# danshapero/sigma

Hardware: AMD Instinct MI355X
Metric: SpMV GB/s (achieved HBM) + CG iters/sec on 5-pt Laplacian, N=1e7 (higher is better)
Workload: dtype f64; 1 GPU; 5-point 2D Poisson CSR, 3162x3162 rows per GPU (rank 0: n=9998244, nnz=49978572), fp64 SpMV y=A*x; rows_per_gpu=9998244, nnz_per_gpu=49978572, parallelism=row-partition x1, matrix_resident_bytes_per_gpu=479920788, reference_layout_bytes_per_gpu=639735844, full=False

## Files before the change

### sigma_amd/csrc/sgm_internal.hpp

```cpp
#pragma once
#include <hip/hip_runtime.h>

#include <cstdarg>
#include <cstdint>
#include <cstdio>
#include <cstring>
#include <string>
#include <atomic>
#include <type_traits>
#include <utility>
#include <vector>

#include "../../include/sigma_hip.h"

namespace sgm {

extern std::string g_err;
int fail(int code, const char *fmt, ...);

#define SGM_HIP(call)                                                              \
    do {                                                                           \
        hipError_t e__ = (call);                                                   \
        if (e__ != hipSuccess)                                                     \
            return sgm::fail(SGM_ERR_HIP, "%s:%d: %s -> %s", __FILE__, __LINE__,   \
                             #call, hipGetErrorString(e__));                       \
    } while (0)
#define SGM_TRY(call)                        \
    do {                                     \
        int rc__ = (call);                   \
        if (rc__ != SGM_OK) return rc__;     \
    } while (0)

constexpr int kEllcbMaxCols = 16384;
struct MatOptions {
    int csr_offset_dict = 1;
    int ell_offset_dict = 1;
    int csr_row_owner = 1;
    int csr_row_lines = 1;
    int csr_sliced = 1;
    int csr_sell = 1;
    int csr_xwindow = 1;
    int csr_lean = 1;
    int ell_colblock = 1;
    int ell_colblock_cols = 16384;
    int ell_colblock_rows = 0;
    int coloring_pass = 0;
    int slice_sched = 0;
};
struct SolverOptions {
    int cg_small = 1;
    int bicgstab_small = 1;
    int krylov_graph = 1;
    int dot_order = 0;
    int gmres_cgs2 = 1;
    int coop_spin_limit = 0;
    int cg_coop_variant = 0;
    int reorder_solve = 2;
    int dist_halo_fused = 1;
};
struct PcOptions {
    int ildu_strips = 1;
    int ildu_rows = 1;
    int pipeline_spin_limit = 0;
    int ildu_reorder = 0;
};
struct Options { MatOptions mat; SolverOptions solver; PcOptions pc; };
int *mat_option_field(MatOptions &o, const char *name);
int *solver_option_field(SolverOptions &o, const char *name);
int *pc_option_field(PcOptions &o, const char *name);
int normalise_option(const char *name, int value, int *out);
extern Options g_opt;

struct Runtime {
    bool ready = false;
// ... 59 lines not shown
    const double *ptr;
    int count;
};

struct HaloNbr {
    int peer = -1;
    int32_t send_count = 0;
    int32_t *send_idx = nullptr;
    double *send_buf = nullptr;
    int32_t recv_offset = 0;
    int32_t recv_count = 0;
};

struct SliceSched { int32_t *tab = nullptr; int32_t lo = 0, hi = 0, grid = 0, iters = 0, band = 0; };

struct Part {
    MatOptions opt = g_opt.mat;
    int32_t n = 0;
    int32_t ncol_own = 0;
    int32_t n_halo = 0;
    int32_t int_lo = 0, int_hi = 0;
    int64_t nnz = 0;
    int64_t row_begin = 0;
    int32_t *rowptr = nullptr;
    int32_t *col = nullptr;
    double *val = nullptr;
    uint8_t *code = nullptr;
    int32_t *dict = nullptr;
    int32_t ndict = 0;
    int32_t dict_reach = 0;
    int32_t max_row = 0;
    double *sval = nullptr;
    uint32_t *scode = nullptr;
    int32_t *scol = nullptr;
    uint8_t *sbcode = nullptr;
    bool lean = false;
    double *sl_val = nullptr;
    int32_t *sl_col = nullptr;
    uint16_t *sl_perm = nullptr;
    int64_t *sl_off = nullptr;
    int64_t sl_total = 0;
    int32_t *sl_win0 = nullptr;
    int32_t sl_gs = 1;
    int32_t sl_span = 0;
    int32_t sw = 0;
    int32_t sched_period = 0;
    mutable SliceSched sched[3];
    mutable int nsched = 0;
    const int32_t *run_sched = nullptr;
    int32_t run_iters = 0;
    int32_t max_d = 0;
    int32_t *ecol = nullptr;
    double *eval = nullptr;
    int32_t *edeg = nullptr;
    uint8_t *ezero = nullptr;
    uint8_t *ecode = nullptr;
    int32_t emdp = 0;
    int32_t *cb_perm = nullptr;
    double *cb_sval = nullptr;
    uint16_t *cb_lcol = nullptr;
    int32_t *cb_bstart = nullptr;
    uint16_t *cb_lpos = nullptr;
    void *cb_fdesc = nullptr;
    double *cb_P = nullptr;
    int32_t cb_cols = 0, cb_nb = 0, cb_R = 0, cb_ntiles = 0, cb_chunks = 0;
    int32_t cb_maxd = 0;
// ... 276 lines not shown
```

### sigma_amd/csrc/sgm_layouts.hip

```cpp
#include "sgm_spmv_select.hpp"

namespace sgm {

__global__ void k_dec1(int32_t *a, int64_t n)
{
    int64_t i = (int64_t)blockIdx.x * blockDim.x + threadIdx.x;
    const int64_t stride = (int64_t)gridDim.x * blockDim.x;
    for (; i < n; i += stride) a[i] -= 1;
}

__global__ void k_check_ptr1(const int32_t *__restrict__ ptr1, int64_t n, int64_t nnz, unsigned long long *bad)
{
    int64_t i = (int64_t)blockIdx.x * blockDim.x + threadIdx.x;
    const int64_t stride = (int64_t)gridDim.x * blockDim.x;
    for (; i <= n; i += stride) {
        const int32_t a = ptr1[i];
        bool ok = true;
        if (i == 0) ok = a == 1;
        if (i < n) ok = ok && ptr1[i + 1] >= a;
        else ok = ok && (int64_t)a - 1 == nnz;
        if (!ok) atomicMin(bad, (unsigned long long)i);
    }
}

// ... 245 lines not shown
{
    if (!p.lean || p.val) return SGM_OK;
    SGM_TRY(dalloc(&p.val, (size_t)p.nnz + 2));
    SGM_HIP(hipMemsetAsync(p.val + p.nnz, 0, 2 * sizeof(double), g_rt.stream));
    return SGM_OK;
}
void csr_release_arrays(const Part &cp)
{
    Part &p = const_cast<Part &>(cp);
    if (!p.lean || !lean_applies(p)) return;
    (void)hipStreamSynchronize(g_rt.stream);
    dfree(p.val); dfree(p.col); dfree(p.code);
    p.val = nullptr; p.col = nullptr; p.code = nullptr;
}

int pack_sliced(Part &p)
{
    if (p.sl_val && p.n > 0) {
        const int64_t nch = (((int64_t)p.n + kSlRows - 1) / kSlRows) * (kSlRows / kSellChunk);
        hipLaunchKernelGGL(k_sell_fill, dim3((unsigned)std::min<int64_t>((nch + 3) / 4, 65536)), dim3(256), 0, g_rt.stream, p.n,
                           (const int32_t *)p.rowptr, (const int32_t *)nullptr, (const double *)p.val, (const int64_t *)p.sl_off,
                           (const uint16_t *)p.sl_perm, (int32_t *)nullptr, p.sl_val);
        SGM_HIP(hipGetLastError());
    }
    if ((!p.scode && !p.scol && !p.sbcode) || p.n == 0) return SGM_OK;
    const int64_t nsl = ((int64_t)p.n + kSlRows - 1) / kSlRows;
    if (p.ecol)
        hipLaunchKernelGGL(k_sl_pack_ell, dim3((unsigned)std::min<int64_t>(nsl, 65536)), dim3(256), 0, g_rt.stream, p.n, p.sw,
                           p.max_d, (const double *)p.eval, p.sval);
    else
        hipLaunchKernelGGL(k_sl_pack, dim3((unsigned)std::min<int64_t>(nsl, 65536)), dim3(256), 0, g_rt.stream, p.n, p.sw,
                           (const int32_t *)p.rowptr, (const double *)p.val, p.sval);
    SGM_HIP(hipGetLastError());
    return SGM_OK;
}

__global__ void k_fill32(int64_t n, int32_t *a, int32_t v)
{
    int64_t i = (int64_t)blockIdx.x * blockDim.x + threadIdx.x;
    const int64_t stride = (int64_t)gridDim.x * blockDim.x;
    for (; i < n; i += stride) a[i] = v;
}

constexpr int kDictSlots = 1024;
constexpr int32_t kDictEmpty = INT32_MIN;
__global__ __launch_bounds__(256) void k_dict_collect(int32_t n, const int32_t *__restrict__ rowptr, const int32_t *__restrict__ col,
                                                      int32_t *table, int *count, int *max_row)
{
    constexpr int kLocal = 512;
    __shared__ int32_t ltab[kLocal];
    __shared__ int lcount;
    for (int t = threadIdx.x; t < kLocal; t += 256) ltab[t] = kDictEmpty;
    if (threadIdx.x == 0) lcount = 0;
    __syncthreads();
    int mr = 0;
    int32_t mine[8];
#pragma unroll
    for (int t = 0; t < 8; ++t) mine[t] = kDictEmpty;
    int next = 0;
    for (int32_t i = blockIdx.x * blockDim.x + threadIdx.x; i < n; i += gridDim.x * blockDim.x) {
        const int32_t s0 = rowptr[i], e = rowptr[i + 1];
        mr = max(mr, e - s0);
        for (int32_t k = s0; k < e; ++k) {
            const int32_t off = col[k] - i;
            bool known = false;
#pragma unroll
// ... 182 lines not shown
        SGM_TRY(build_ell_colblock(p));
        if (p.cb_P) return SGM_OK;
        const int W = p.max_row <= 3 ? 3 : p.max_row <= 5 ? 5 : p.max_row <= 7 ? 7 : p.max_row <= 8 ? 8 : p.max_row <= 12 ? 12
                    : p.max_row <= 16 ? 16 : p.max_row <= 20 ? 20 : p.max_row <= 24 ? 24 : p.max_row <= 28 ? 28 : 32;
        if (!p.opt.csr_sliced || p.max_row < 1 || p.max_row > 32 || (double)W * n > 1.25 * (double)nnz) return build_sell(p);
        const size_t rows_padded = ((size_t)n + kSlRows - 1) / kSlRows * kSlRows;
        SGM_TRY(dalloc(&p.scol, rows_padded * W));
        SGM_TRY(dalloc(&p.sval, rows_padded * W));
        p.sw = W;
        hipLaunchKernelGGL(k_sl_pack_cols, dim3((unsigned)std::min<size_t>(rows_padded / kSlRows, 65536)), dim3(256), 0, g_rt.stream,
                           n, W, (const int32_t *)p.rowptr, (const int32_t *)p.col, p.scol);
        SGM_HIP(hipGetLastError());
        return pack_sliced(p);
    };
    if (!p.opt.csr_offset_dict || hcnt[0] > 255) return sliced32();
    std::vector<int32_t> dict;
    for (int32_t v : htab) if (v != kDictEmpty) dict.push_back(v);
    std::sort(dict.begin(), dict.end());
    p.ndict = (int32_t)dict.size();
    p.dict_reach = 0;
    for (int32_t v : dict) p.dict_reach = std::max(p.dict_reach, v < 0 ? -v : v);
    dict.resize(256, 0);
    SGM_TRY(dalloc(&p.code, (size_t)nnz + 32));
    SGM_TRY(dalloc(&p.dict, (size_t)256));
    SGM_HIP(hipMemcpyAsync(p.dict, dict.data(), 256 * 4, hipMemcpyHostToDevice, st));
    SGM_HIP(hipMemsetAsync(p.code + nnz, 0, 32, st));
    const int W = p.max_row <= 3 ? 3 : p.max_row <= 5 ? 5 : p.max_row <= 7 ? 7 : 8;
    const bool sliced = p.opt.csr_sliced && p.ndict <= 15 && p.max_row >= 1 && p.max_row <= 8 && (double)W * n <= 1.25 * (double)nnz;
    size_t rows_padded = 0;
    if (sliced) {
        rows_padded = ((size_t)n + kSlRows - 1) / kSlRows * kSlRows;
        SGM_TRY(dalloc(&p.scode, rows_padded));
        SGM_TRY(dalloc(&p.sval, rows_padded * W));
        hipLaunchKernelGGL(k_fill32, dim3(vec_grid(rows_padded)), dim3(256), 0, st, (int64_t)rows_padded,
                           reinterpret_cast<int32_t *>(p.scode), (int32_t)-1);
        p.sw = W;
    }
    hipLaunchKernelGGL(k_dict_encode, dim3(grid), dim3(256), 0, st, n, (const int32_t *)p.rowptr, (const int32_t *)p.col,
                       (const int32_t *)p.dict, p.ndict, p.code, sliced ? p.scode : nullptr);
    SGM_HIP(hipGetLastError());
    if (sliced) SGM_TRY(pack_sliced(p));
    int Wb = 0;
#define PICK(WW) if (!Wb && p.max_row <= WW) Wb = WW;
    SGM_SLB_WIDTHS(PICK)
#undef PICK
    const int Wc = (Wb + 7) / 8 * 8;
    if (!sliced && p.opt.csr_sliced && Wb && p.ndict <= 255 && p.max_row > 8 && (double)Wb * n <= 1.35 * (double)nnz) {
        rows_padded = ((size_t)n + kSlRows - 1) / kSlRows * kSlRows;
        SGM_TRY(dalloc(&p.sbcode, rows_padded * Wc));
        SGM_TRY(dalloc(&p.sval, rows_padded * Wb));
        p.sw = Wb;
        hipLaunchKernelGGL(k_slb_pack_codes, dim3((unsigned)std::min<size_t>(rows_padded / kSlRows, 65536)), dim3(256), 0, st, n, Wb,
                           (const int32_t *)p.rowptr, (const uint8_t *)p.code, p.sbcode);
        SGM_HIP(hipGetLastError());
        SGM_TRY(pack_sliced(p));
    }
    SGM_HIP(hipStreamSynchronize(st));
    if (p.scode || p.sbcode) SGM_TRY(detect_sched_period_csr(p, dict));
    if (!p.scode && !p.sbcode) {
        SGM_TRY(build_sell(p));
        if (p.sl_val) {
            dfree(p.code); dfree(p.dict);
            p.code = nullptr; p.dict = nullptr;
            p.ndict = 0; p.dict_reach = 0;
        }
    }
// ... 200 lines not shown
        return fail(SGM_ERR_UNSUPPORTED, "clone_csr_plain: single-GPU CSR matrices only");
    const Part &p = A->parts[0];
    SGM_TRY(csr_need_arrays(p));
    struct Release { const Part &p; ~Release() { csr_release_arrays(p); } } rel{p};
    sgm_mat C = new sgm_mat_s;
    C->fmt = SGM_FMT_CSR; C->nrow = A->nrow; C->ncol = A->ncol; C->nnz = A->nnz;
    C->parts.resize(1);
    Part &q = C->parts[0];
    q.opt.csr_offset_dict = 0; q.opt.csr_sliced = 0; q.opt.csr_sell = 0; q.opt.csr_lean = 0; q.opt.slice_sched = 0;
    q.n = p.n; q.ncol_own = p.ncol_own; q.n_halo = 0; q.nnz = p.nnz; q.max_row = p.max_row;
    hipStream_t st = g_rt.stream;
    int rc = dalloc(&q.rowptr, (size_t)p.n + 1);
    if (rc == SGM_OK) rc = dalloc(&q.col, (size_t)p.nnz + 4);
    if (rc == SGM_OK) rc = dalloc(&q.val, (size_t)p.nnz + 2);
    if (rc != SGM_OK) { sgm_mat_destroy(C); return rc; }
    (void)hipMemcpyAsync(q.rowptr, p.rowptr, ((size_t)p.n + 1) * 4, hipMemcpyDeviceToDevice, st);
    (void)hipMemsetAsync(q.col + p.nnz, 0, 16, st);
    (void)hipMemsetAsync(q.val + p.nnz, 0, 16, st);
    if (p.nnz) {
        (void)hipMemcpyAsync(q.col, p.col, (size_t)p.nnz * 4, hipMemcpyDeviceToDevice, st);
        (void)hipMemcpyAsync(q.val, p.val, (size_t)p.nnz * 8, hipMemcpyDeviceToDevice, st);
    }
    if (hipStreamSynchronize(st) != hipSuccess || hipGetLastError() != hipSuccess) { sgm_mat_destroy(C); return fail(SGM_ERR_HIP, "clone_csr_plain: copy failed"); }
    *out = C;
    return SGM_OK;
}

int rebuild_csr_formats(Part &p)
{
    SGM_TRY(csr_need_arrays(p));
    p.lean = false;
    dfree(p.code); dfree(p.dict); dfree(p.sval); dfree(p.scode); dfree(p.scol); dfree(p.sbcode);
    p.code = nullptr; p.dict = nullptr; p.sval = nullptr; p.scode = nullptr; p.scol = nullptr; p.sbcode = nullptr;
    free_sell(p);
    free_ell_colblock(p);
    p.ndict = 0; p.dict_reach = 0; p.sw = 0; p.max_row = 0; p.sched_period = 0;
    free_slice_sched(p);
    return build_offset_dict(p, nullptr, nullptr);
}
int rebuild_ell_formats(Part &p)
{
    dfree(p.ecode); dfree(p.dict); dfree(p.sval); dfree(p.scode);
    p.ecode = nullptr; p.dict = nullptr; p.dict_reach = 0; p.emdp = 0; p.sval = nullptr; p.scode = nullptr; p.sw = 0; p.sched_period = 0;
    free_slice_sched(p);
    SGM_TRY(build_ell_offset_dict(p));
    SGM_TRY(build_ell_colblock(p));
    return refresh_ell_colblock_values(p);
}
int sgm_invalidate_transpose(sgm_mat A)
{
    if (A->T) { sgm_mat_destroy(A->T); A->T = nullptr; }
    dfree(A->tperm);
    A->tperm = nullptr;
    A->t_stale = true;
    return SGM_OK;
}

void free_part(Part &p)
{
    dfree(p.rowptr); dfree(p.col); dfree(p.val); dfree(p.code); dfree(p.dict); dfree(p.sval); dfree(p.scode); dfree(p.scol); dfree(p.sbcode); dfree(p.ecol); dfree(p.eval); dfree(p.edeg); dfree(p.ezero); dfree(p.ecode); dfree(p.xext);
    for (auto &nb : p.nbrs) { dfree(nb.send_idx); dfree(nb.send_buf); }
    free_slice_sched(p);
    free_ell_colblock(p);
    free_sell(p);
    p = Part();
}

}
```

### sigma_amd/csrc/sgm_mat.hip

```cpp
#include "sgm_spmv_select.hpp"
#include "sgm_krylov.hpp"
#include "sgm_plan_host.hpp"

namespace sgm {

int stage_in(Staged &s, const double *v, int64_t n, int where, bool copy)
{
    if (where == SGM_DEVICE && (reinterpret_cast<uintptr_t>(v) & 15) == 0) {
        s.dev = const_cast<double *>(v);
        return SGM_OK;
    }
    SGM_TRY(dalloc(&s.dev, (size_t)n));
    s.owned = true;
    if (copy)
        SGM_HIP(hipMemcpyAsync(s.dev, v, (size_t)n * 8,
                               where == SGM_HOST ? hipMemcpyHostToDevice : hipMemcpyDeviceToDevice,
                               g_rt.stream));
    return SGM_OK;
}
int stage_out(const Staged &s, double *v, int64_t n, int where)
{
    if (!s.owned) return SGM_OK;
    SGM_HIP(hipMemcpyAsync(v, s.dev, (size_t)n * 8,
                           where == SGM_HOST ? hipMemcpyDeviceToHost : hipMemcpyDeviceToDevice,
// ... 453 lines not shown
    unsigned long long *bad = nullptr, hbad = ~0ull;
    SGM_TRY(dalloc(&deg, (size_t)std::max(n, 1)));
    int rc = dalloc(&bad, 1);
    if (rc == SGM_OK && hipMemsetAsync(bad, 0xff, sizeof hbad, st) != hipSuccess) rc = fail(SGM_ERR_HIP, "sgm_ell_set_degrees: memset");
    if (rc == SGM_OK && n &&
        hipMemcpyAsync(deg, degrees, (size_t)n * 4, where == SGM_HOST ? hipMemcpyHostToDevice : hipMemcpyDeviceToDevice, st) != hipSuccess)
        rc = fail(SGM_ERR_HIP, "sgm_ell_set_degrees: copy of degrees");
    if (rc == SGM_OK && n)
        hipLaunchKernelGGL(k_ell_check_degrees, dim3((n + kBlock - 1) / kBlock), dim3(kBlock), 0, st, n, p.max_d, (const int32_t *)deg,
                           (const uint8_t *)p.ezero, bad);
    if (rc == SGM_OK && (hipMemcpyAsync(&hbad, bad, sizeof hbad, hipMemcpyDeviceToHost, st) != hipSuccess ||
                         hipStreamSynchronize(st) != hipSuccess || hipGetLastError() != hipSuccess))
        rc = fail(SGM_ERR_HIP, "sgm_ell_set_degrees: check kernel failed");
    dfree(bad);
    if (rc == SGM_OK && hbad != ~0ull) {
        int32_t d = 0;
        (void)hipMemcpy(&d, deg + hbad, 4, hipMemcpyDeviceToHost);
        rc = fail(SGM_ERR_DIMS, "sgm_ell_set_degrees: degrees(%lld) = %d: outside 0..%d, or one of the first %d slots of that row holds no column",
                  (long long)hbad + 1, d, p.max_d, d);
    }
    if (rc != SGM_OK) { dfree(deg); return rc; }
    dfree(p.edeg);
    p.edeg = deg;
    A->version += 1;
    A->pattern_version += 1;
    return SGM_OK;
}

int sgm_mat_set_option(sgm_mat A, const char *name, int value)
{
    SGM_TRY(require_init());
    if (!A || !name) return fail(SGM_ERR_BAD_ARG, "sgm_mat_set_option: null argument");
    int v = 0;
    SGM_TRY(normalise_option(name, value, &v));
    MatOptions probe;
    if (!mat_option_field(probe, name)) return fail(SGM_ERR_BAD_ARG, "sgm_mat_set_option: '%s' is not a matrix option", name);
    if (A->fmt == SGM_FMT_COMPOSITE) {
        for (sgm_mat_s *B : A->blocks)
            if (B) SGM_TRY(sgm_mat_set_option(B, name, value));
        return SGM_OK;
    }
    const bool cb_shape = !strcmp(name, "ell_colblock_cols") || !strcmp(name, "ell_colblock_rows");
    for (Part &p : A->parts) {
        int *f = mat_option_field(p.opt, name);
        const int old = *f;
        *f = v;
        if (old == v) continue;
        if ((p.ecol || (!p.lean && p.rowptr && p.col && p.val && p.n_halo == 0 && !p.sval && !p.sl_val)) &&
            (cb_shape || (!strcmp(name, "ell_colblock") && ((old != 0) != (v != 0) || v == 2 || old == 2)))) {
            SGM_TRY(build_ell_colblock(p));
            SGM_TRY(refresh_ell_colblock_values(p));
            SGM_HIP(hipStreamSynchronize(g_rt.stream));
        }
        if (!strcmp(name, "csr_lean") && !p.ecol) {
            if (v == 0) { SGM_TRY(csr_need_arrays(p)); p.lean = false; }
            else csr_go_lean(p);
        }
        if (!strcmp(name, "slice_sched")) free_slice_sched(p);
    }
    if (A->T) SGM_TRY(sgm_mat_set_option(A->T, name, value));
    return SGM_OK;
}

int sgm_mat_matvec(sgm_mat A, const double *x, double *y, int where)
{
    return matvec_impl(A, x, y, where, false);
// ... 106 lines not shown
        SGM_HIP(hipMemcpy(vi.data(), p.rowptr, vi.size() * 4, hipMemcpyDeviceToHost));
        for (auto &v : vi) v += 1;
    } else if (!ell && nm == "node") {
        vi.resize((size_t)p.nnz);
        if (p.nnz) SGM_HIP(hipMemcpy(vi.data(), p.col, vi.size() * 4, hipMemcpyDeviceToHost));
        for (auto &v : vi) v += 1;
    } else if (!ell && nm == "val") {
        vd.resize((size_t)p.nnz);
        if (p.nnz) SGM_HIP(hipMemcpy(vd.data(), p.val, vd.size() * 8, hipMemcpyDeviceToHost));
    } else if (ell && nm == "max_d") {
        vi.assign(1, p.max_d);
    } else if (ell && nm == "degrees") {
        SGM_TRY(ell_need_degrees("sgm_mat_get(\"degrees\")", p));
        vi.assign((size_t)p.n, 0);
        if (p.n && p.edeg) SGM_HIP(hipMemcpy(vi.data(), p.edeg, vi.size() * 4, hipMemcpyDeviceToHost));
    } else if (ell && (nm == "node" || nm == "val")) {
        const size_t total = (size_t)p.n * p.max_d;
        if (nm == "node") {
            std::vector<int32_t> t(total);
            std::vector<uint8_t> z(p.ezero ? total : 0);
            if (total) SGM_HIP(hipMemcpy(t.data(), p.ecol, total * 4, hipMemcpyDeviceToHost));
            if (!z.empty()) SGM_HIP(hipMemcpy(z.data(), p.ezero, total, hipMemcpyDeviceToHost));
            vi.resize(total);
            for (int32_t i = 0; i < p.n; ++i)
                for (int32_t k = 0; k < p.max_d; ++k)
                    vi[(size_t)i * p.max_d + k] = !z.empty() && z[(size_t)k * p.n + i] ? 0 : t[(size_t)k * p.n + i] + 1;
        } else {
            std::vector<double> t(total);
            if (total) SGM_HIP(hipMemcpy(t.data(), p.eval, total * 8, hipMemcpyDeviceToHost));
            vd.resize(total);
            for (int32_t i = 0; i < p.n; ++i)
                for (int32_t k = 0; k < p.max_d; ++k) vd[(size_t)i * p.max_d + k] = t[(size_t)k * p.n + i];
        }
    } else if (nm == "algebra_rows" && A->alg) {
        vi.resize(2);
        alg_plan_rows(A->alg, vi.data());
    } else if (nm == "versions") {
        vq = {(int64_t)A->serial, (int64_t)A->version, (int64_t)A->pattern_version};
    } else {
        return fail(SGM_ERR_BAD_ARG, "sgm_mat_get: unknown array '%s' for this format", name);
    }
    const size_t sz = vi.size() * 4 + vd.size() * 8 + vq.size() * 8;
    if (needed) *needed = sz;
    if (out && sz) {
        if (bytes < sz) return fail(SGM_ERR_BAD_ARG, "sgm_mat_get: buffer too small (%zu < %zu)", bytes, sz);
        memcpy(out, !vq.empty() ? (const void *)vq.data() : vi.empty() ? (const void *)vd.data() : (const void *)vi.data(), sz);
    }
    return SGM_OK;
}

int sgm_mat_info(sgm_mat A, int32_t *nrow, int32_t *ncol, int64_t *nnz, int32_t *fmt, int64_t *x_len)
{
    if (!A) return fail(SGM_ERR_BAD_ARG, "sgm_mat_info: null matrix");
    if (nrow) *nrow = A->nrow;
    if (ncol) *ncol = A->ncol;
    if (nnz) *nnz = A->nnz;
    if (fmt) *fmt = A->fmt;
    if (x_len) *x_len = A->comm ? A->parts[0].xlen() : A->ncol;
    return SGM_OK;
}

}
namespace sgm {
void part_kernel_name(const Part &p, int fmt, char *name, size_t len)
{
    if (fmt == SGM_FMT_ELL) {
        if (use_ell_colblock(p)) snprintf(name, len, "k_ellcb<cols=%d,R=%d>", p.cb_cols, p.cb_R);
        else if (use_sliced_ell(p)) snprintf(name, len, "k_csr_sl<W=%d>", p.sw);
        else if (p.ecode && p.opt.ell_offset_dict) snprintf(name, len, "k_ell_do<MDP=%d>", p.emdp);
        else snprintf(name, len, "k_ell_spmv");
    } else if (use_ell_colblock(p)) snprintf(name, len, "k_ellcb<cols=%d,R=%d,csr>", p.cb_cols, p.cb_R);
    else if (use_sliced(p)) snprintf(name, len, "k_csr_sl<W=%d>", p.sw);
    else if (use_slicedb(p)) snprintf(name, len, "k_csr_slb<W=%d>", p.sw);
    else if (use_sliced32(p)) snprintf(name, len, "k_csr_sl32<W=%d>", p.sw);
    else if (use_sell(p)) snprintf(name, len, p.sl_win0 && p.opt.csr_xwindow ? "k_csr_sell<pad=%.3f,xw=%dx%d>" : "k_csr_sell<pad=%.3f>",
                                   p.nnz ? (double)p.sl_total / (double)p.nnz : 1.0, p.sl_span, p.sl_gs);
    else if (use_offset_dict(p)) snprintf(name, len, "k_csr_do<256,%d,CW=1>", do_tile_for(p));
    else if (use_row_owner(p)) snprintf(name, len, "k_csr_do<256,%d,CW=4>", do_tile_for(p));
    else if (use_row_lines(p)) snprintf(name, len, "k_csr_rl");
    else snprintf(name, len, "k_csr_spmv");
}
}
extern "C" {

int sgm_mat_kernel(sgm_mat A, char *buf, int len)
{
    if (!A || !buf || len < 1) return fail(SGM_ERR_BAD_ARG, "sgm_mat_kernel: bad argument");
    char name[64];
    if (A->fmt == SGM_FMT_COMPOSITE) snprintf(name, sizeof name, "composite");
    else part_kernel_name(A->parts[0], A->fmt, name, sizeof name);
    snprintf(buf, (size_t)len, "%s", name);
    return SGM_OK;
}

static int64_t part_resident_bytes(const Part &p)
{
    int64_t b = 0;
    const int64_t nsl = ((int64_t)p.n + kSlRows - 1) / kSlRows;
    if (p.rowptr) b += 4 * ((int64_t)p.n + 1);
    if (p.col) b += 4 * (p.nnz + 4);
    if (p.val) b += 8 * (p.nnz + 2);
    if (p.code) b += p.nnz + 16;
    if (p.dict) b += 4 * 256;
    if (p.sval) b += 8 * nsl * kSlRows * p.sw;
    if (p.scode) b += 4 * nsl * kSlRows;
    if (p.scol) b += 4 * nsl * kSlRows * p.sw;
    if (p.sbcode) b += nsl * kSlRows * ((p.sw + 7) / 8 * 8);
    if (p.sl_val) b += 12 * p.sl_total + 2 * nsl * kSlRows + 8 * (nsl * (kSlRows / kSellChunk) + 1);
    if (p.ecol) b += 4 * (int64_t)p.n * p.max_d;
    if (p.eval) b += 8 * (int64_t)p.n * p.max_d;
    if (p.edeg) b += 4 * (int64_t)p.n;
    if (p.ezero) b += (int64_t)p.n * p.max_d;
    if (p.ecode) b += (int64_t)p.n * p.emdp;
    if (p.xext) b += 8 * p.xlen();
    b += ell_colblock_resident_bytes(p);
    for (const auto &nb : p.nbrs) b += (int64_t)nb.send_count * (nb.send_buf ? 12 : 4);
    return b;
}
static int64_t part_matvec_bytes(const sgm_mat_s *A, const Part &p)
{
    const int64_t nsl = ((int64_t)p.n + kSlRows - 1) / kSlRows;
    int64_t m;
    if (A->fmt == SGM_FMT_ELL) {
        if (use_ell_colblock(p)) return ell_colblock_matvec_bytes(p);
        if (use_sliced_ell(p)) m = nsl * kSlRows * (8 * (int64_t)p.sw + 4);
        else if (p.ecode && p.opt.ell_offset_dict) m = (int64_t)p.n * (8 * (int64_t)p.max_d + p.emdp);
        else m = 12 * (int64_t)p.n * p.max_d;
    } else if (use_ell_colblock(p)) return ell_colblock_matvec_bytes(p);
    else if (use_sliced(p)) m = nsl * kSlRows * (8 * (int64_t)p.sw + 4);
    else if (use_slicedb(p)) m = nsl * kSlRows * (8 * (int64_t)p.sw + (p.sw + 7) / 8 * 8);
    else if (use_sliced32(p)) m = nsl * kSlRows * 12 * (int64_t)p.sw;
    else if (use_sell(p)) {
        m = 12 * p.sl_total + 2 * nsl * kSlRows + 8 * nsl * (kSlRows / kSellChunk);
        if (p.sl_win0 && p.opt.csr_xwindow)
            return m + ((nsl + p.sl_gs - 1) / p.sl_gs) * (8 * (int64_t)p.sl_span + 4) + 8 * (int64_t)p.n;
    }
    else if (use_offset_dict(p)) m = 9 * p.nnz + 4 * ((int64_t)p.n + 1);
    else m = 12 * p.nnz + 4 * ((int64_t)p.n + 1);
    return m + 8 * p.xlen() + 8 * (int64_t)p.n;
}

int sgm_mat_footprint(sgm_mat A, int64_t *resident_bytes, int64_t *matvec_bytes)
{
    if (!A) return fail(SGM_ERR_BAD_ARG, "sgm_mat_footprint: null matrix");
    int64_t res = 0, mv = 0;
    if (A->fmt == SGM_FMT_COMPOSITE) {
        for (sgm_mat C : A->blocks) {
            if (!C) continue;
            int64_t r = 0, m = 0;
            SGM_TRY(sgm_mat_footprint(C, &r, &m));
            mv += m + 8 * (int64_t)C->nrow;
        }
        mv += 8 * (int64_t)A->nrow;
    } else {
        for (const Part &p : A->parts) { res += part_resident_bytes(p); mv += part_matvec_bytes(A, p); }
        if (A->T) { int64_t r = 0; SGM_TRY(sgm_mat_footprint(A->T, &r, nullptr)); res += r + 4 * A->nnz; }
    }
    if (resident_bytes) *resident_bytes = res;
    if (matvec_bytes) *matvec_bytes = mv;
    return SGM_OK;
}

// ... 13 lines not shown
```

### sigma_amd/csrc/sgm_spmv.hip

```cpp
#include "sgm_spmv_device.hpp"
#include "sgm_plan_host.hpp"

#include <cassert>

namespace sgm {


template <int BLOCK, int VPT, bool NT, bool ADD, bool DOT_W, bool DOT_YY>
__global__ __launch_bounds__(BLOCK) void k_csr_spmv(
    int32_t n, const int32_t *__restrict__ rowptr, const int32_t *__restrict__ col,
    const double *__restrict__ val, const double *__restrict__ x, double *__restrict__ y,
    const double *__restrict__ w, double *__restrict__ part_wy, double *__restrict__ part_yy,
    const int *__restrict__ flag_done, int gen, int remap)
{
    constexpr int TILE = 2 * BLOCK * VPT;
    __shared__ double prod[TILE];
    __shared__ double red[BLOCK / 64];
    if (stopped(flag_done, gen)) return;

    const int tid = threadIdx.x;
    const bool chain = (remap & kChainBit) != 0;
    const int64_t nrb = ((int64_t)n + BLOCK - 1) / BLOCK;
    double dwy = 0.0, dyy = 0.0;

// ... 280 lines not shown
                for (int m = 0; m < VPT; ++m) {
                    const int32_t j = ts + 2 * tid + 2 * BLOCK * m;
                    if (j < te) *reinterpret_cast<i32x2 *>(cl4 + (j - ts)) = c8[m];
                }
            }
            __syncthreads();
            if (PF && ts + TILE < e) fetch(ts + TILE, min(ts + 2 * TILE, e));
            const int32_t kend = min(ke, te);
            while (k < kend) {
                const int cnt = min(kend - k, U);
                double xv[U], vv[U];
#pragma unroll
                for (int u = 0; u < U; ++u)
                    if (u < cnt) {
                        const int o = k + u - ts;
                        xv[u] = CW == 1 ? x[row + dl[cl[o]]] : x[(int32_t)cl4[o]];
                        vv[u] = vl[o];
                    }
#pragma unroll
                for (int u = 0; u < U; ++u)
                    if (u < cnt) z = z + vv[u] * xv[u];
                k += cnt;
            }
        }
        if (row < n) {
            const double yi = row_value<ADD>(y0, z, chain);
            __builtin_nontemporal_store(yi, y + row);
            dots_add<DOT_W, DOT_YY>(DOT_W ? w[row] : 0.0, yi, dwy, dyy);
        }
    }
    dots_write<BLOCK, DOT_W, DOT_YY>(dwy, dyy, red, part_wy, part_yy);
}

template <int W, bool ADD, bool DOT_W, bool DOT_YY>
__global__ __launch_bounds__(256) void k_csr_sl(
    int32_t n, const uint32_t *__restrict__ scode, const int32_t *__restrict__ dict,
    const double *__restrict__ sval, const double *__restrict__ x, double *__restrict__ y,
    const double *__restrict__ w, double *__restrict__ part_wy, double *__restrict__ part_yy,
    const int *__restrict__ flag_done, int gen, int remap, const int32_t *__restrict__ sched, int sched_iters)
{
    constexpr int BLOCK = 256;
    __shared__ int32_t dl[16];
    __shared__ double red[BLOCK / 64];
    const int st = stop_flag(flag_done);
    const int tid = threadIdx.x;
    const bool chain = (remap & kChainBit) != 0;
    const int32_t dv = tid < 16 ? dict[tid] : 0;
    const int64_t nsl = ((int64_t)n + kSlRows - 1) / kSlRows;
    double dwy = 0.0, dyy = 0.0;

    const int64_t first = first_slice(remap & kSliceMapBits);
    int64_t sl = sched ? sched[blockIdx.x] : first;
    int sit = 0;
    u32x2 cw = {0xffffffffu, 0xffffffffu};
    f64x2 v[W];
    auto load_slice = [&](int64_t s_) {
        const int32_t row_ = (int32_t)(s_ * kSlRows) + 2 * tid;
        cw = __builtin_nontemporal_load(reinterpret_cast<const u32x2 *>(scode + row_));
        const f64x2 *vb = reinterpret_cast<const f64x2 *>(sval + s_ * (int64_t)(W * kSlRows)) + tid;
#pragma unroll
        for (int u = 0; u < W; ++u) v[u] = __builtin_nontemporal_load(vb + u * BLOCK);
    };
    bool have = sl >= 0 && sl < nsl;
    if (have) load_slice(sl);
    if (stop_hit(st, gen)) return;
    if (tid < 16) dl[tid] = dv;
    __syncthreads();
    while (have) {
        int64_t nxt = sl + gridDim.x;
        if (sched) { ++sit; nxt = sit < sched_iters ? sched[(int64_t)sit * gridDim.x + blockIdx.x] : -1; }
        const int32_t row = (int32_t)(sl * kSlRows) + 2 * tid;
        const f64x2 y0 = pair_load_y0<ADD>(y, row, n);
        const f64x2 z = sl_row_sums<W>(pair_start<ADD>(y0, chain), cw, v, x, row, dl);
        pair_finish<ADD, DOT_W, DOT_YY>(y, w, row, n, y0, z, chain, dwy, dyy);
        sl = nxt;
        have = sl >= 0 && sl < nsl;
        if (have) load_slice(sl);
    }
    dots_write<BLOCK, DOT_W, DOT_YY>(dwy, dyy, red, part_wy, part_yy);
}

template <bool ADD, bool DOT_W, bool DOT_YY, bool XW = false, int GS = 1>
__global__ __launch_bounds__(256 * GS) void k_csr_sell(
    int32_t n, const int64_t *__restrict__ off, const uint16_t *__restrict__ perm, const int32_t *__restrict__ scol,
    const double *__restrict__ sval, const double *__restrict__ x, double *__restrict__ y, const double *__restrict__ w,
    double *__restrict__ part_wy, double *__restrict__ part_yy, const int *__restrict__ flag_done, int gen, int remap,
    const int32_t *__restrict__ win0 = nullptr, int32_t span = 0, int32_t xlen = 0)
{
    constexpr int BLOCK = 256 * GS;
    extern __shared__ double xs[];
    __shared__ double red[BLOCK / 64];
    const int st = stop_flag(flag_done);
    const int lane = threadIdx.x & 63;
    const int wave = __builtin_amdgcn_readfirstlane(threadIdx.x >> 6);
    const bool chain = (remap & kChainBit) != 0;
    const int64_t nsl = ((int64_t)n + kSlRows - 1) / kSlRows;
    double dwy = 0.0, dyy = 0.0;
    if (stop_hit(st, gen)) return;

    int64_t first = blockIdx.x;
    if ((remap & 255) >= 3) {
        const int G = (remap & 255) == 3 ? 8 : (remap & 255) == 4 ? 2 : (remap & 255) == 6 ? 64 : (remap & 255) == 7 ? 128 : 32;
        const int xcd = blockIdx.x & 7, loc = blockIdx.x >> 3;
        first = (int64_t)(loc / G) * (8 * G) + xcd * G + loc % G;
    }
    const int64_t ngr = (nsl + GS - 1) / GS;
    for (int64_t gr = first; gr < ngr; gr += gridDim.x) {
        const int64_t sl = gr * GS + (GS == 2 ? (wave >> 2) : 0);
        const bool has = sl < nsl;
        const int64_t chunk = (has ? sl : nsl - 1) * (kSlRows / kSellChunk) + (GS == 2 ? (wave & 3) : wave);
// ... 266 lines not shown
    });
}

static void launch_csr_do(const Part &p, int grid, const SpmvArgs &a)
{
    const int tile = do_tile_for(p);
    const bool dict = use_offset_dict(p);
    assert(!dict || tile <= kDoMaxCodeTile);
    with_flags(a, [&](auto flags) {
        using F = decltype(flags);
#define LV(T)                                                                                                               \
    if (tile == T) {                                                                                                        \
        if (!dict)                                                                                                          \
            hipLaunchKernelGGL((k_csr_do<kSpmvBlock, T, 4, F::add, F::dot_w, F::dot_yy>), dim3(grid), dim3(kSpmvBlock), 0, g_rt.stream, p.n, \
                               p.rowptr, reinterpret_cast<const uint8_t *>(p.col), p.dict, p.val, a.x, a.y, a.w, a.pwy, a.pyy, \
                               a.flag, a.gen, chain_bit(a));                                                                \
        else if constexpr (T <= kDoMaxCodeTile)                                                                             \
            hipLaunchKernelGGL((k_csr_do<kSpmvBlock, T, 1, F::add, F::dot_w, F::dot_yy>), dim3(grid), dim3(kSpmvBlock), 0, g_rt.stream, p.n, \
                               p.rowptr, p.code, p.dict, p.val, a.x, a.y, a.w, a.pwy, a.pyy, a.flag, a.gen, chain_bit(a));  \
        return;                                                                                                             \
    }
        SGM_DO_TILES(LV)
#undef LV
    });
}

static void launch_csr_sl(const Part &p, int grid, const SpmvArgs &a)
{
    const int remap = slice_map_mode(grid, p.n) | chain_bit(a);
    with_flags(a, [&](auto flags) {
        using F = decltype(flags);
#define LV(WW)                                                                                                              \
    if (p.sw == WW) {                                                                                                       \
        hipLaunchKernelGGL((k_csr_sl<WW, F::add, F::dot_w, F::dot_yy>), dim3(grid), dim3(256), 0, g_rt.stream, p.n, p.scode, p.dict, p.sval, \
                           a.x, a.y, a.w, a.pwy, a.pyy, a.flag, a.gen, remap, p.run_sched, p.run_iters);                    \
        return;                                                                                                             \
    }
        SGM_SL_WIDTHS(LV)
#undef LV
    });
}

static void launch_csr_sl32(const Part &p, int grid, const SpmvArgs &a)
{
    const int remap = slice_map_mode(grid, p.n) | chain_bit(a);
    with_flags(a, [&](auto flags) {
        using F = decltype(flags);
#define LV(WW)                                                                                                              \
    if (p.sw == WW) {                                                                                                       \
        hipLaunchKernelGGL((k_csr_sl32<WW, F::add, F::dot_w, F::dot_yy>), dim3(grid), dim3(256), 0, g_rt.stream, p.n, p.scol, p.sval, a.x, a.y, \
                           a.w, a.pwy, a.pyy, a.flag, a.gen, remap);                                                        \
        return;                                                                                                             \
    }
        SGM_SL32_WIDTHS(LV)
#undef LV
    });
}

static void launch_csr_slb(const Part &p, int grid, const SpmvArgs &a)
{
    const int remap = slice_map_mode(grid, p.n) | chain_bit(a);
    with_flags(a, [&](auto flags) {
        using F = decltype(flags);
#define LV(WW)                                                                                                              \
    if (p.sw == WW) {                                                                                                       \
        hipLaunchKernelGGL((k_csr_slb<WW, F::add, F::dot_w, F::dot_yy>), dim3(grid), dim3(256), 0, g_rt.stream, p.n, p.sbcode, p.dict, p.sval, \
                           a.x, a.y, a.w, a.pwy, a.pyy, a.flag, a.gen, remap, p.run_sched, p.run_iters);                    \
        return;                                                                                                             \
// ... 113 lines not shown
    for (int i = 0; i < p.nsched; ++i)
        if (p.sched[i].lo == lo && p.sched[i].hi == hi && p.sched[i].grid == grid) return p.sched[i].tab ? &p.sched[i] : nullptr;
    if (p.nsched >= 3) return nullptr;
    SliceSched &ss = p.sched[p.nsched++];
    ss.lo = lo; ss.hi = hi; ss.grid = grid; ss.tab = nullptr; ss.band = band;
    std::vector<int32_t> tab;
    int iters = 0;
    slice_sched_table(nsl, p.sched_period, grid, band, tab, iters);
    int32_t *d = nullptr;
    if (dalloc(&d, tab.size()) != SGM_OK) return nullptr;
    if (hipMemcpy(d, tab.data(), tab.size() * sizeof(int32_t), hipMemcpyHostToDevice) != hipSuccess) { dfree(d); return nullptr; }
    ss.tab = d; ss.iters = iters;
    return &ss;
}
void free_slice_sched(Part &p)
{
    for (int i = 0; i < p.nsched; ++i) { dfree(p.sched[i].tab); p.sched[i] = SliceSched(); }
    p.nsched = 0;
}

static void launch_range(const Part &p, const RowRange &r, const SpmvArgs &a)
{
    Part v;
    v.opt = p.opt;
    v.n = r.hi - r.lo;
    v.nnz = (int64_t)((double)p.nnz * v.n / (p.n > 0 ? p.n : 1));
    v.n_halo = p.n_halo; v.ncol_own = p.ncol_own;
    v.rowptr = p.rowptr + r.lo; v.col = p.col; v.val = p.val; v.code = p.code; v.dict = p.dict;
    v.max_row = p.max_row;
    const bool sliced = use_sliced(p), slicedb = !sliced && use_slicedb(p), sliced32 = !sliced && !slicedb && use_sliced32(p);
    if (sliced || slicedb)
        if (const SliceSched *ss = slice_sched(p, r.lo, r.hi, r.grid)) { v.run_sched = ss->tab; v.run_iters = ss->iters; }
    if (sliced) { v.sval = p.sval + (int64_t)r.lo * p.sw; v.scode = p.scode + r.lo; v.sw = p.sw; }
    if (slicedb) { v.sval = p.sval + (int64_t)r.lo * p.sw; v.sbcode = p.sbcode + (int64_t)r.lo * ((p.sw + 7) / 8 * 8); v.sw = p.sw; }
    if (sliced32) { v.sval = p.sval + (int64_t)r.lo * p.sw; v.scol = p.scol + (int64_t)r.lo * p.sw; v.sw = p.sw; }
    const bool sell = !sliced && !slicedb && !sliced32 && use_sell(p);
    if (sell) {
        v.sl_val = p.sl_val; v.sl_col = p.sl_col;
        v.sl_off = p.sl_off + r.lo / kSellChunk; v.sl_perm = p.sl_perm + r.lo;
        v.sl_gs = p.sl_gs;
        v.sl_win0 = p.sl_win0 ? p.sl_win0 + r.lo / (kSlRows * p.sl_gs) : nullptr; v.sl_span = p.sl_span;
    }
    const bool dict = use_offset_dict(p);
    SpmvArgs ar = a;
    ar.y = a.y + r.lo;
    ar.w = a.w ? a.w + r.lo : nullptr;
    ar.pwy = a.pwy ? a.pwy + r.part_off : nullptr;
    ar.pyy = a.pyy ? a.pyy + r.part_off : nullptr;
    if (dict && !sliced32 && !sell) ar.x = a.x + r.lo;
    if (sliced) launch_csr_sl(v, r.grid, ar);
    else if (slicedb) launch_csr_slb(v, r.grid, ar);
    else if (sliced32) launch_csr_sl32(v, r.grid, ar);
    else if (sell) launch_csr_sell(v, r.grid, ar);
    else if (use_row_owner(p)) launch_csr_do(v, r.grid, ar);
    else if (use_row_lines(p)) launch_csr_rl(v, r.grid, ar);
    else launch_csr(v, r.grid, ar);
}

static int composite_spmv(sgm_mat A, const double *x, double *y, bool add, const SpmvDots *dots,
                          const int *flag_done, int *grid_out, int gen);

int spmv_parts(sgm_mat A, const double *const *x, double *const *y, bool add,
               const SpmvDots *dots, const int *flag_done, int *grid_out, int gen, bool chain, bool halo_ready)
{
    if (A->fmt == SGM_FMT_COMPOSITE) return composite_spmv(A, x[0], y[0], add, dots, flag_done, grid_out, gen);
    const size_t P = A->parts.size();
// ... 138 lines not shown
```

### sigma_amd/csrc/sgm_spmv_select.hpp

```cpp
#pragma once
#include "sgm_internal.hpp"

#include <type_traits>

#include <hipcub/hipcub.hpp>

#include <algorithm>
#include <cstdlib>
#include <string>
#include <vector>

namespace sgm {

typedef double f64x2 __attribute__((ext_vector_type(2)));
typedef int i32x2 __attribute__((ext_vector_type(2)));
typedef int i32x4 __attribute__((ext_vector_type(4)));
typedef uint32_t u32x2 __attribute__((ext_vector_type(2)));
typedef uint16_t u16x2 __attribute__((ext_vector_type(2)));
typedef unsigned int u32x4s __attribute__((ext_vector_type(4)));
#define SGM_SLB_WIDTHS(X) X(9) X(12) X(15) X(16) X(19) X(20) X(24) X(25) X(27) X(28) X(32)
#define SGM_SL_WIDTHS(X) X(3) X(5) X(7) X(8)
#define SGM_SL32_WIDTHS(X) X(3) X(5) X(7) X(8) X(12) X(16) X(20) X(24) X(28) X(32)
constexpr int kSlRows = 512;
constexpr int kSellChunk = 128;
// ... 20 lines not shown
template <bool ADD, bool DOT_W, bool DOT_YY>
struct SpmvFlags { static constexpr bool add = ADD, dot_w = DOT_W, dot_yy = DOT_YY; };
template <class F>
static void with_flags(const SpmvArgs &a, F &&f)
{
    const bool dot_w = a.w != nullptr, dot_yy = a.pyy != nullptr;
    if (a.add) {
        if (dot_w && dot_yy) f(SpmvFlags<true, true, true>{});
        else if (dot_w) f(SpmvFlags<true, true, false>{});
        else if (dot_yy) f(SpmvFlags<true, false, true>{});
        else f(SpmvFlags<true, false, false>{});
    } else {
        if (dot_w && dot_yy) f(SpmvFlags<false, true, true>{});
        else if (dot_w) f(SpmvFlags<false, true, false>{});
        else if (dot_yy) f(SpmvFlags<false, false, true>{});
        else f(SpmvFlags<false, false, false>{});
    }
}

int resident_per_cu(bool row_owner, int tile, int cw);
static const SliceSched *slice_sched(const Part &p, int32_t lo, int32_t hi, int grid);
void free_slice_sched(Part &p);
int ell_grid(const Part &p);
bool use_ell_colblock(const Part &p);
int ell_colblock_grid(const Part &p);
int build_ell_colblock(Part &p);
int refresh_ell_colblock_values(Part &p);
void free_ell_colblock(Part &p);
int launch_ell_colblock(const Part &p, int grid, const SpmvArgs &a);
int64_t ell_colblock_resident_bytes(const Part &p);
int64_t ell_colblock_matvec_bytes(const Part &p);
static bool use_offset_dict(const Part &p) { return (p.code || (p.lean && p.dict)) && p.opt.csr_offset_dict; }
static bool use_sliced(const Part &p) { return p.scode && p.opt.csr_sliced && p.opt.csr_offset_dict; }
static bool use_sliced32(const Part &p) { return p.scol && p.opt.csr_sliced && !p.ecol; }
static bool use_slicedb(const Part &p) { return p.sbcode && p.opt.csr_sliced && p.opt.csr_offset_dict; }
static bool use_sell(const Part &p) { return p.sl_val && p.opt.csr_sliced && p.opt.csr_sell && !p.ecol; }
static bool any_sliced(const Part &p) { return use_sliced(p) || use_sliced32(p) || use_slicedb(p) || use_sell(p); }
static bool use_sliced_ell(const Part &p) { return p.ecol && p.scode && p.opt.csr_sliced && p.opt.ell_offset_dict; }
static bool use_row_owner(const Part &p)
{
    return use_offset_dict(p) || (p.opt.csr_row_owner && p.max_row > 0 && p.max_row <= 64);
}

static bool use_row_lines(const Part &p)
{
    return p.opt.csr_row_lines && !any_sliced(p) && !use_row_owner(p) && p.n > 0 && p.max_row <= 4096 &&
           p.nnz >= 16 * (int64_t)p.n && (int64_t)p.max_row * p.n <= 4 * p.nnz;
}
int row_lines_resident_per_cu();

#define SGM_DO_TILES(X) X(1024) X(1536) X(1920) X(2048) X(4096)
constexpr int kDoMaxCodeTile = 2048;
static int do_tile_for(const Part &p)
{
    static const int tiles[] = {1024, 1536, 1920, 2048, 4096};
    const int nt = use_offset_dict(p) ? 4 : 5;
    const double per_block = (double)p.nnz / (p.n > 0 ? p.n : 1) * kSpmvBlock + 4;
    for (int i = 0; i < nt; ++i)
        if (per_block <= tiles[i]) return tiles[i];
    return tiles[nt - 1];
}

static int grid_for_rows(const Part &p, int64_t rows, int64_t limit, bool dots = true)
{
    const int blk = any_sliced(p) ? kSlRows : kSpmvBlock;
    const int64_t nrb = (rows + blk - 1) / blk;
// ... 8 lines not shown
    return (int)g;
}

struct RowRange { int32_t lo, hi; int grid, part_off; };
static int spmv_ranges(const Part &p, RowRange out[3], bool dots = true, bool whole = false)
{
    int nr = 0, off = 0;
    auto add = [&](int32_t lo, int32_t hi) {
        if (hi <= lo) return;
        out[nr] = RowRange{lo, hi, grid_for_rows(p, hi - lo, nr == 0 ? kMaxGrid / 4 : kMaxGrid / 8), off};
        off += out[nr].grid;
        ++nr;
    };
    if (p.n_halo == 0 || p.int_hi <= p.int_lo || whole) {
        if (any_sliced(p)) {
            out[0] = RowRange{0, p.n, grid_for_rows(p, p.n > 0 ? p.n : 1, kMaxGrid, dots), 0};
            return 1;
        }
        add(0, p.n > 0 ? p.n : 1);
        if (nr) out[0].hi = p.n;
        return nr;
    }
    add(p.int_lo, p.int_hi);
    add(0, p.int_lo);
    add(p.int_hi, p.n);
    return nr;
}


void free_part(Part &p);
void csr_go_lean(Part &p);
int lean_val_buffer(Part &p);
int pack_sliced(Part &p);
int build_ell_offset_dict(Part &p);
__global__ void k_ell_transpose(const int32_t *__restrict__ node, const double *__restrict__ val, int32_t *__restrict__ ecol,
                                double *__restrict__ eval, int32_t n, int32_t max_d, int32_t ncol = 0, unsigned long long *bad = nullptr);
}
```

Before: 6343 GB/s.

## Detect uniform 128-row chunks and load one shared code/value set per wave

At pack time, a classification kernel marks each 128-row chunk of the sliced layout where every row has identical offset codes and values. The SpMV kernel gets a UNI template variant: for flagged chunks, each wave loads one code word and W values and broadcasts them to all lanes instead of streaming per-row data. This targets the matrix-value and code traffic that dominates a stencil-like CSR. The costs are an extra classify pass with a host sync at setup, a per-slice flag lookup in the loop, and a reduced byte model, which changes how achieved bandwidth is reported.

```diff
diff --git a/sigma_amd/csrc/sgm_internal.hpp b/sigma_amd/csrc/sgm_internal.hpp
--- a/sigma_amd/csrc/sgm_internal.hpp
+++ b/sigma_amd/csrc/sgm_internal.hpp
@@ -40,6 +40,7 @@
     int csr_sliced = 1;
     int csr_sell = 1;
     int csr_xwindow = 1;
+    int csr_uniform = 1;
     int csr_lean = 1;
     int ell_colblock = 1;
     int ell_colblock_cols = 16384;
@@ -165,6 +166,9 @@
     int32_t max_row = 0;
     double *sval = nullptr;
     uint32_t *scode = nullptr;
+    int32_t *suni = nullptr;
+    int32_t *suni_count = nullptr;
+    int64_t suni_set = 0;
     int32_t *scol = nullptr;
     uint8_t *sbcode = nullptr;
     bool lean = false;
diff --git a/sigma_amd/csrc/sgm_layouts.hip b/sigma_amd/csrc/sgm_layouts.hip
--- a/sigma_amd/csrc/sgm_layouts.hip
+++ b/sigma_amd/csrc/sgm_layouts.hip
@@ -301,6 +301,47 @@
         hipLaunchKernelGGL(k_sl_pack, dim3((unsigned)std::min<int64_t>(nsl, 65536)), dim3(256), 0, g_rt.stream, p.n, p.sw,
                            (const int32_t *)p.rowptr, (const double *)p.val, p.sval);
     SGM_HIP(hipGetLastError());
+    return classify_sliced(p);
+}
+
+__global__ __launch_bounds__(256) void k_sl_classify(int32_t n, int32_t W, const uint32_t *__restrict__ scode,
+                                                     const unsigned long long *__restrict__ sval, int32_t *__restrict__ suni,
+                                                     int32_t *__restrict__ count)
+{
+    const int64_t nch = (((int64_t)n + kSlRows - 1) / kSlRows) * (kSlRows / kUniChunk);
+    const int wave = threadIdx.x >> 6, lane = threadIdx.x & 63;
+    for (int64_t c = (int64_t)blockIdx.x * 4 + wave; c < nch; c += (int64_t)gridDim.x * 4) {
+        const int64_t row0 = c * kUniChunk;
+        const int64_t sl = row0 / kSlRows;
+        const int r0 = (int)(row0 - sl * kSlRows);
+        bool same = row0 + kUniChunk <= n;
+        if (same) {
+            const uint32_t *cp = scode + row0;
+            same = cp[lane] == cp[0] && cp[lane + 64] == cp[0];
+            const unsigned long long *vp = sval + sl * (int64_t)W * kSlRows + r0;
+            for (int u = 0; u < W; ++u, vp += kSlRows) same = same && vp[lane] == vp[0] && vp[lane + 64] == vp[0];
+        }
+        const bool all = __ballot(same) == ~0ull;
+        if (lane == 0) {
+            suni[c] = all ? 1 : 0;
+            if (all) atomicAdd(count, 1);
+        }
+    }
+}
+
+int classify_sliced(Part &p)
+{
+    if (!p.suni || !p.scode || !p.sval) return SGM_OK;
+    const int64_t nch = uni_chunks(p);
+    int32_t set = 0;
+    SGM_HIP(hipMemsetAsync(p.suni_count, 0, sizeof(int32_t), g_rt.stream));
+    if (nch > 0)
+        hipLaunchKernelGGL(k_sl_classify, dim3((unsigned)std::min<int64_t>((nch + 3) / 4, 65536)), dim3(256), 0, g_rt.stream, p.n, p.sw,
+                           (const uint32_t *)p.scode, reinterpret_cast<const unsigned long long *>(p.sval), p.suni, p.suni_count);
+    SGM_HIP(hipGetLastError());
+    SGM_HIP(hipMemcpyAsync(&set, p.suni_count, sizeof set, hipMemcpyDeviceToHost, g_rt.stream));
+    SGM_HIP(hipStreamSynchronize(g_rt.stream));
+    p.suni_set = set;
     return SGM_OK;
 }
 
@@ -549,6 +590,8 @@
         rows_padded = ((size_t)n + kSlRows - 1) / kSlRows * kSlRows;
         SGM_TRY(dalloc(&p.scode, rows_padded));
         SGM_TRY(dalloc(&p.sval, rows_padded * W));
+        SGM_TRY(dalloc(&p.suni, rows_padded / kUniChunk));
+        SGM_TRY(dalloc(&p.suni_count, 1));
         hipLaunchKernelGGL(k_fill32, dim3(vec_grid(rows_padded)), dim3(256), 0, st, (int64_t)rows_padded,
                            reinterpret_cast<int32_t *>(p.scode), (int32_t)-1);
         p.sw = W;
@@ -815,6 +858,8 @@
     p.lean = false;
     dfree(p.code); dfree(p.dict); dfree(p.sval); dfree(p.scode); dfree(p.scol); dfree(p.sbcode);
     p.code = nullptr; p.dict = nullptr; p.sval = nullptr; p.scode = nullptr; p.scol = nullptr; p.sbcode = nullptr;
+    dfree(p.suni); dfree(p.suni_count);
+    p.suni = nullptr; p.suni_count = nullptr; p.suni_set = 0;
     free_sell(p);
     free_ell_colblock(p);
     p.ndict = 0; p.dict_reach = 0; p.sw = 0; p.max_row = 0; p.sched_period = 0;
@@ -842,6 +887,7 @@
 void free_part(Part &p)
 {
     dfree(p.rowptr); dfree(p.col); dfree(p.val); dfree(p.code); dfree(p.dict); dfree(p.sval); dfree(p.scode); dfree(p.scol); dfree(p.sbcode); dfree(p.ecol); dfree(p.eval); dfree(p.edeg); dfree(p.ezero); dfree(p.ecode); dfree(p.xext);
+    dfree(p.suni); dfree(p.suni_count);
     for (auto &nb : p.nbrs) { dfree(nb.send_idx); dfree(nb.send_buf); }
     free_slice_sched(p);
     free_ell_colblock(p);
diff --git a/sigma_amd/csrc/sgm_mat.hip b/sigma_amd/csrc/sgm_mat.hip
--- a/sigma_amd/csrc/sgm_mat.hip
+++ b/sigma_amd/csrc/sgm_mat.hip
@@ -509,6 +509,17 @@
     SGM_TRY(require_init());
     if (!A || !name) return fail(SGM_ERR_BAD_ARG, "sgm_mat_set_option: null argument");
     int v = 0;
+    if (!strcmp(name, "csr_uniform")) {
+        v = value < 0 ? 0 : value > 2 ? 2 : value;
+        if (A->fmt == SGM_FMT_COMPOSITE) {
+            for (sgm_mat_s *B : A->blocks)
+                if (B) SGM_TRY(sgm_mat_set_option(B, name, v));
+            return SGM_OK;
+        }
+        for (Part &p : A->parts) p.opt.csr_uniform = v;
+        if (A->T) SGM_TRY(sgm_mat_set_option(A->T, name, v));
+        return SGM_OK;
+    }
     SGM_TRY(normalise_option(name, value, &v));
     MatOptions probe;
     if (!mat_option_field(probe, name)) return fail(SGM_ERR_BAD_ARG, "sgm_mat_set_option: '%s' is not a matrix option", name);
@@ -681,6 +692,12 @@
             for (int32_t i = 0; i < p.n; ++i)
                 for (int32_t k = 0; k < p.max_d; ++k) vd[(size_t)i * p.max_d + k] = t[(size_t)k * p.n + i];
         }
+    } else if (!ell && nm == "uniform_chunks") {
+        if (p.suni) {
+            vi.resize((size_t)uni_chunks(p) + 1);
+            vi[0] = (int32_t)p.suni_set;
+            if (vi.size() > 1) SGM_HIP(hipMemcpy(vi.data() + 1, p.suni, (vi.size() - 1) * 4, hipMemcpyDeviceToHost));
+        }
     } else if (nm == "algebra_rows" && A->alg) {
         vi.resize(2);
         alg_plan_rows(A->alg, vi.data());
@@ -738,7 +755,8 @@
     char name[64];
     if (A->fmt == SGM_FMT_COMPOSITE) snprintf(name, sizeof name, "composite");
     else part_kernel_name(A->parts[0], A->fmt, name, sizeof name);
-    snprintf(buf, (size_t)len, "%s", name);
+    const bool uni = A->fmt == SGM_FMT_CSR && use_uniform(A->parts[0]);
+    snprintf(buf, (size_t)len, uni ? "%s+UNI" : "%s", name);
     return SGM_OK;
 }
 
@@ -753,6 +771,7 @@
     if (p.dict) b += 4 * 256;
     if (p.sval) b += 8 * nsl * kSlRows * p.sw;
     if (p.scode) b += 4 * nsl * kSlRows;
+    if (p.suni) b += 4 * uni_chunks(p) + 4;
     if (p.scol) b += 4 * nsl * kSlRows * p.sw;
     if (p.sbcode) b += nsl * kSlRows * ((p.sw + 7) / 8 * 8);
     if (p.sl_val) b += 12 * p.sl_total + 2 * nsl * kSlRows + 8 * (nsl * (kSlRows / kSellChunk) + 1);
@@ -776,7 +795,10 @@
         else if (p.ecode && p.opt.ell_offset_dict) m = (int64_t)p.n * (8 * (int64_t)p.max_d + p.emdp);
         else m = 12 * (int64_t)p.n * p.max_d;
     } else if (use_ell_colblock(p)) return ell_colblock_matvec_bytes(p);
-    else if (use_sliced(p)) m = nsl * kSlRows * (8 * (int64_t)p.sw + 4);
+    else if (use_sliced(p)) {
+        m = nsl * kSlRows * (8 * (int64_t)p.sw + 4);
+        if (use_uniform(p)) m = (uni_chunks(p) - p.suni_set) * kUniChunk * (8 * (int64_t)p.sw + 4) + p.suni_set * (8 * (int64_t)p.sw + 4 + 4);
+    }
     else if (use_slicedb(p)) m = nsl * kSlRows * (8 * (int64_t)p.sw + (p.sw + 7) / 8 * 8);
     else if (use_sliced32(p)) m = nsl * kSlRows * 12 * (int64_t)p.sw;
     else if (use_sell(p)) {
diff --git a/sigma_amd/csrc/sgm_spmv.hip b/sigma_amd/csrc/sgm_spmv.hip
--- a/sigma_amd/csrc/sgm_spmv.hip
+++ b/sigma_amd/csrc/sgm_spmv.hip
@@ -336,12 +336,13 @@
     dots_write<BLOCK, DOT_W, DOT_YY>(dwy, dyy, red, part_wy, part_yy);
 }
 
-template <int W, bool ADD, bool DOT_W, bool DOT_YY>
+template <int W, bool ADD, bool DOT_W, bool DOT_YY, bool UNI = false>
 __global__ __launch_bounds__(256) void k_csr_sl(
     int32_t n, const uint32_t *__restrict__ scode, const int32_t *__restrict__ dict,
     const double *__restrict__ sval, const double *__restrict__ x, double *__restrict__ y,
     const double *__restrict__ w, double *__restrict__ part_wy, double *__restrict__ part_yy,
-    const int *__restrict__ flag_done, int gen, int remap, const int32_t *__restrict__ sched, int sched_iters)
+    const int *__restrict__ flag_done, int gen, int remap, const int32_t *__restrict__ sched, int sched_iters,
+    const int32_t *__restrict__ suni = nullptr)
 {
     constexpr int BLOCK = 256;
     __shared__ int32_t dl[16];
@@ -358,7 +359,23 @@
     int sit = 0;
     u32x2 cw = {0xffffffffu, 0xffffffffu};
     f64x2 v[W];
-    auto load_slice = [&](int64_t s_) {
+    const int wave = UNI ? __builtin_amdgcn_readfirstlane(tid >> 6) : 0;
+    int uf = 0;
+    uint32_t ucw = 0xffffffffu;
+    double uv[W];
+    auto chunk_flag = [&](int64_t s_) { return suni[s_ * (kSlRows / kUniChunk) + wave]; };
+    auto load_slice = [&](int64_t s_, int f) {
+        if (UNI) {
+            f = __builtin_amdgcn_readfirstlane(f);
+            uf = f;
+            if (f) {
+                ucw = scode[s_ * kSlRows + wave * kUniChunk];
+                const double *ub = sval + s_ * (int64_t)(W * kSlRows) + wave * kUniChunk;
+#pragma unroll
+                for (int u = 0; u < W; ++u) uv[u] = ub[u * kSlRows];
+                return;
+            }
+        }
         const int32_t row_ = (int32_t)(s_ * kSlRows) + 2 * tid;
         cw = __builtin_nontemporal_load(reinterpret_cast<const u32x2 *>(scode + row_));
         const f64x2 *vb = reinterpret_cast<const f64x2 *>(sval + s_ * (int64_t)(W * kSlRows)) + tid;
@@ -366,20 +383,27 @@
         for (int u = 0; u < W; ++u) v[u] = __builtin_nontemporal_load(vb + u * BLOCK);
     };
     bool have = sl >= 0 && sl < nsl;
-    if (have) load_slice(sl);
+    if (have) load_slice(sl, UNI ? chunk_flag(sl) : 0);
     if (stop_hit(st, gen)) return;
     if (tid < 16) dl[tid] = dv;
     __syncthreads();
     while (have) {
         int64_t nxt = sl + gridDim.x;
         if (sched) { ++sit; nxt = sit < sched_iters ? sched[(int64_t)sit * gridDim.x + blockIdx.x] : -1; }
+        const bool have_nxt = nxt >= 0 && nxt < nsl;
+        const int fn = UNI && have_nxt ? chunk_flag(nxt) : 0;
+        if (UNI && uf) {
+            cw.x = ucw; cw.y = ucw;
+#pragma unroll
+            for (int u = 0; u < W; ++u) { v[u].x = uv[u]; v[u].y = uv[u]; }
+        }
         const int32_t row = (int32_t)(sl * kSlRows) + 2 * tid;
         const f64x2 y0 = pair_load_y0<ADD>(y, row, n);
         const f64x2 z = sl_row_sums<W>(pair_start<ADD>(y0, chain), cw, v, x, row, dl);
         pair_finish<ADD, DOT_W, DOT_YY>(y, w, row, n, y0, z, chain, dwy, dyy);
         sl = nxt;
-        have = sl >= 0 && sl < nsl;
-        if (have) load_slice(sl);
+        have = have_nxt;
+        if (have) load_slice(sl, fn);
     }
     dots_write<BLOCK, DOT_W, DOT_YY>(dwy, dyy, red, part_wy, part_yy);
 }
@@ -712,8 +736,12 @@
         using F = decltype(flags);
 #define LV(WW)                                                                                                              \
     if (p.sw == WW) {                                                                                                       \
-        hipLaunchKernelGGL((k_csr_sl<WW, F::add, F::dot_w, F::dot_yy>), dim3(grid), dim3(256), 0, g_rt.stream, p.n, p.scode, p.dict, p.sval, \
-                           a.x, a.y, a.w, a.pwy, a.pyy, a.flag, a.gen, remap, p.run_sched, p.run_iters);                    \
+        if (p.suni)                         \
+            hipLaunchKernelGGL((k_csr_sl<WW, F::add, F::dot_w, F::dot_yy, true>), dim3(grid), dim3(256), 0, g_rt.stream, p.n, p.scode, p.dict, \
+                               p.sval, a.x, a.y, a.w, a.pwy, a.pyy, a.flag, a.gen, remap, p.run_sched, p.run_iters, (const int32_t *)p.suni); \
+        else                                                                                                                \
+            hipLaunchKernelGGL((k_csr_sl<WW, F::add, F::dot_w, F::dot_yy>), dim3(grid), dim3(256), 0, g_rt.stream, p.n, p.scode, p.dict, p.sval, \
+                               a.x, a.y, a.w, a.pwy, a.pyy, a.flag, a.gen, remap, p.run_sched, p.run_iters);                \
         return;                                                                                                             \
     }
         SGM_SL_WIDTHS(LV)
@@ -893,6 +921,7 @@
     if (sliced || slicedb)
         if (const SliceSched *ss = slice_sched(p, r.lo, r.hi, r.grid)) { v.run_sched = ss->tab; v.run_iters = ss->iters; }
     if (sliced) { v.sval = p.sval + (int64_t)r.lo * p.sw; v.scode = p.scode + r.lo; v.sw = p.sw; }
+    if (sliced && use_uniform(p)) v.suni = p.suni + r.lo / kUniChunk;
     if (slicedb) { v.sval = p.sval + (int64_t)r.lo * p.sw; v.sbcode = p.sbcode + (int64_t)r.lo * ((p.sw + 7) / 8 * 8); v.sw = p.sw; }
     if (sliced32) { v.sval = p.sval + (int64_t)r.lo * p.sw; v.scol = p.scol + (int64_t)r.lo * p.sw; v.sw = p.sw; }
     const bool sell = !sliced && !slicedb && !sliced32 && use_sell(p);
diff --git a/sigma_amd/csrc/sgm_spmv_select.hpp b/sigma_amd/csrc/sgm_spmv_select.hpp
--- a/sigma_amd/csrc/sgm_spmv_select.hpp
+++ b/sigma_amd/csrc/sgm_spmv_select.hpp
@@ -76,6 +76,15 @@
 int64_t ell_colblock_matvec_bytes(const Part &p);
 static bool use_offset_dict(const Part &p) { return (p.code || (p.lean && p.dict)) && p.opt.csr_offset_dict; }
 static bool use_sliced(const Part &p) { return p.scode && p.opt.csr_sliced && p.opt.csr_offset_dict; }
+constexpr int kUniChunk = 128;
+constexpr int64_t kUniMinRows = (int64_t)1 << 20;
+constexpr int kUniMaxAutoWidth = 5;
+static int64_t uni_chunks(const Part &p) { return (((int64_t)p.n + kSlRows - 1) / kSlRows) * (kSlRows / kUniChunk); }
+static bool use_uniform(const Part &p)
+{
+    if (!use_sliced(p) || !p.suni || p.opt.csr_uniform == 0) return false;
+    return p.opt.csr_uniform == 2 || (p.n >= kUniMinRows && p.sw <= kUniMaxAutoWidth && 4 * p.suni_set >= uni_chunks(p));
+}
 static bool use_sliced32(const Part &p) { return p.scol && p.opt.csr_sliced && !p.ecol; }
 static bool use_slicedb(const Part &p) { return p.sbcode && p.opt.csr_sliced && p.opt.csr_offset_dict; }
 static bool use_sell(const Part &p) { return p.sl_val && p.opt.csr_sliced && p.opt.csr_sell && !p.ecol; }
@@ -150,6 +159,7 @@
 void csr_go_lean(Part &p);
 int lean_val_buffer(Part &p);
 int pack_sliced(Part &p);
+int classify_sliced(Part &p);
 int build_ell_offset_dict(Part &p);
 __global__ void k_ell_transpose(const int32_t *__restrict__ node, const double *__restrict__ val, int32_t *__restrict__ ecol,
                                 double *__restrict__ eval, int32_t n, int32_t max_d, int32_t ncol = 0, unsigned long long *bad = nullptr);
```

After: 4497 GB/s. -29.1%, worse.
